# HongwenZhang/DaNet-DensePose2SMPL

Hardware: AMD Instinct MI355X
Metric: images/sec fwd+bwd HRNet-W48+SMPL+IUV 256x256 bs32/GPU (higher is better)
Workload: dtype bf16; 1 GPU; full DaNet train step (HRNet-W48 + global and part-wise IUV heads + regressor nets + SMPL LBS (2 forward + 1 backward; the 2 label-side forwards belong to the untimed batch prologue) + IUV render + losses, fwd+bwd+Adam), 256x256, 32 img/GPU; convs bf16 MFMA fp32-acc, LBS/raster/losses fp32; global_batch=32, parallelism=dp1

## Files before the change

danet-densepose2smpl_amd/_lib.py:

```python
import ctypes
import os

_HERE = os.path.dirname(os.path.abspath(__file__))
LIB_PATH = os.environ.get('DANET_LIB') or os.path.join(_HERE, 'csrc', 'libdanet_hip.so')
_lib = None

c_f = ctypes.c_void_p
c_i = ctypes.c_int
c_sz = ctypes.c_size_t
c_fl = ctypes.c_float

_SIGNATURES = {
    'danet_version': (c_i, []),
    'danet_last_error': (ctypes.c_char_p, []),
    'danet_smpl_lbs_debug': (c_i, [c_f]),
    'danet_smpl_lbs_ctx_floats': (c_sz, [c_i]),
    'danet_smpl_lbs_fwd_ws_floats': (c_sz, [c_i, c_i, c_i]),
    'danet_smpl_lbs_bwd_ws_floats': (c_sz, [c_i, c_i, c_i]),
    'danet_smpl_lbs_ticket_words': (c_sz, [c_i]),
    'danet_smpl_lbs_forward': (c_i, [c_f, c_f, c_i] + [c_f] * 9 + [c_i] * 4 + [c_f] * 5 + [c_sz, c_f, c_f]),
    'danet_smpl_lbs_backward': (c_i, [c_f, c_f, c_i] + [c_f] * 7 + [c_i] * 4 + [c_f] * 7 + [c_sz, c_f, c_i, c_f]),
    'danet_smpl_lbs_backward_fused_ok': (c_i, [c_i, c_i, c_i]),
    'danet_iuv_raster_ws_bytes': (c_sz, [c_i, c_i, c_i]),
    'danet_iuv_raster_forward': (c_i, [c_f, c_f, c_i, c_i, c_f, c_i, c_f, c_f, c_i, c_fl, c_fl, c_i, c_f, c_f, c_f, c_f, c_sz, c_f]),
# ... 44 lines not shown
    'danet_conv_wgrad3x3_pair_ok': (c_i, [c_i] * 11),
    'danet_conv_wgrad3x3_ws_floats': (c_sz, [c_i] * 7),
    'danet_conv_wgrad_multi_ws_floats': (c_sz, [c_f, c_i]),
    'danet_conv_wgrad_multi_ws_zero_from': (c_sz, [c_f, c_i]),
    'danet_conv_wgrad_multi': (c_i, [c_f, c_i, c_f, c_sz, c_fl, c_f]),
    'danet_conv_wgrad3x3_multi_ws_floats': (c_sz, [c_f, c_i]),
    'danet_conv_wgrad3x3_multi': (c_i, [c_f, c_i, c_f, c_sz, c_fl, c_f]),
    'danet_conv_wgrad3x3_kernel_id': (c_i, [c_i] * 7),
    'danet_conv_wgrad3x3': (c_i, [c_f] * 4 + [c_sz] + [c_i] * 7 + [c_fl, c_i, c_f]),
    'danet_conv_wgrad_ws_floats': (c_sz, [c_i] * 4),
    'danet_conv_wgrad_ws_floats_for': (c_sz, [c_i] * 13),
    'danet_conv_wgrad': (c_i, [c_f] * 4 + [c_sz] + [c_i] * 13 + [c_fl, c_i, c_f]),
    'danet_bn_forward': (c_i, [c_f, c_f, c_f, ctypes.c_int64, c_i] + [c_f] * 6 + [c_i, c_fl, c_fl, c_i, c_i, c_f, c_f]),
    'danet_bn_ws_floats': (c_sz, [c_i]),
    'danet_knob': (ctypes.c_long, [c_i, ctypes.c_long]),
    'danet_bn_acc_bytes': (c_i, []),
    'danet_channel_sum': (c_i, [c_f, ctypes.c_int64, c_i, c_f, c_i, c_i, c_f]),
    'danet_bn_forward_multi': (c_i, [c_f, c_i, c_fl, c_fl, c_f]),
    'danet_bn_backward_multi': (c_i, [c_f, c_i, c_f]),
    'danet_bn_backward_onepass_ok': (c_i, [c_f, c_i, c_i]),
    'danet_bn_backward_onepass_bar_words': (c_i, []),
    'danet_bn_backward_onepass': (c_i, [c_f, c_i, c_f, c_i, c_f]),
    'danet_bn_backward': (c_i, [c_f, c_f, c_f, ctypes.c_int64, c_i, c_f, c_f, c_i, c_f, c_f, c_f, c_f, c_i, c_i, c_f, c_f, c_f]),
    'danet_sum_relu_forward': (c_i, [ctypes.POINTER(ctypes.c_void_p), ctypes.POINTER(c_i), c_i, c_i, c_i, c_i, c_i, c_i, c_f, c_f]),
    'danet_sum_relu_backward': (c_i, [c_f, c_f, c_i, c_i, c_i, c_i, c_i, c_i, c_f, c_f]),
    'danet_sum_relu_backward_all': (c_i, [c_f, c_f] + [c_i] * 5 + [c_f] * 5),
    'danet_sum_relu_forward_multi': (c_i, [c_f, c_i, c_f]),
    'danet_sum_relu_backward_all_multi': (c_i, [c_f, c_i, c_f]),
    'danet_maxpool3x3s2_forward': (c_i, [c_f, c_f, c_f, c_i, c_i, c_i, c_i, c_f]),
    'danet_maxpool3x3s2_backward': (c_i, [c_f, c_f, c_f, c_i, c_i, c_i, c_i, c_f]),
    'danet_stn_gather_forward': (c_i, [c_f, c_f] + [c_i] * 8 + [c_f, c_f]),
    'danet_stn_gather_backward': (c_i, [c_f, c_f] + [c_i] * 8 + [c_f, c_f]),
    'danet_part_clean_forward': (c_i, [c_f, c_f, c_i, c_i, c_i, c_i, c_f, c_f]),
    'danet_part_clean_backward': (c_i, [c_f, c_f, c_f, c_i, c_i, c_i, c_i, c_f, c_f]),
    'danet_part_loss_forward': (c_i, [c_f] * 5 + [c_i] * 5 + [c_f, c_f]),
    'danet_part_loss_backward': (c_i, [c_f] * 6 + [c_i] * 5 + [c_f, c_f]),
    'danet_part_backward_fused': (c_i, [c_f] * 8 + [c_i] * 5 + [c_f, c_f]),
    'danet_part_gt_forward': (c_i, [c_f] * 5 + [c_i] * 4 + [c_f, c_f, c_f]),
    'danet_part_gt_backward': (c_i, [c_f] * 5 + [c_i] * 4 + [c_f, c_f]),
    'danet_iuv_global_forward': (c_i, [c_f] * 4 + [c_i, c_i] + [c_f] * 3 + [c_i] * 4 + [c_f] * 5),
    'danet_iuv_global_backward': (c_i, [c_f] * 4 + [c_i, c_i] + [c_f] * 6 + [c_i] * 4 + [c_f] * 5),
    'danet_softargmax_forward': (c_i, [c_f, c_i, c_i, c_i, c_i, c_i, c_fl, c_f, c_f, c_f]),
    'danet_softargmax_backward': (c_i, [c_f, c_i, c_i, c_i, c_i, c_i, c_fl, c_f, c_f, c_f, c_f]),
    'danet_dp_point_losses_rows': (c_i, [c_i, c_i]),
    'danet_dp_point_losses_forward': (c_i, [c_f] * 4 + [c_i, c_i] + [c_f] * 8 + [c_i] * 3 + [c_f, c_f]),
    'danet_dp_point_losses_backward': (c_i, [c_f] * 4 + [c_i, c_i] + [c_f] * 9 + [c_i] * 3 + [c_f] * 5),
# ... 259 lines not shown
```

danet-densepose2smpl_amd/csrc/build.py:

```python
import os
import subprocess
import sys
from concurrent.futures import ThreadPoolExecutor

HERE = os.path.dirname(os.path.abspath(__file__))
ROOT = os.path.dirname(os.path.dirname(HERE))
LIB = os.path.join(HERE, 'libdanet_hip.so')
ARCH = 'gfx950'

MFMA_VGPR = ['-mllvm', '-amdgpu-mfma-vgpr-form']
UNITS = {
    'capi.hip': [],
    'smpl_lbs.hip': [],
    'iuv_raster.hip': ['-ffp-contract=off'],
    'geometry.hip': [],
    'conv_igemm.hip': MFMA_VGPR,
    'conv_wgrad.hip': MFMA_VGPR,
    'conv_wgrad3x3.hip': MFMA_VGPR,
    'conv_wgrad_rows.hip': MFMA_VGPR,
    'conv3x3.hip': MFMA_VGPR,
    'conv3x3s.hip': MFMA_VGPR,
    'conv_fast.hip': MFMA_VGPR,
    'conv_g3.hip': MFMA_VGPR,
    'conv_pw.hip': MFMA_VGPR,
    'conv_pw_wgrad.hip': MFMA_VGPR,
    'conv3x3a.hip': [],
    'conv_stem_dgrad.hip': [],
    'conv_stem.hip': [],
    'conv_f32.hip': ['-ffp-contract=off'],
    'conv_f32m.hip': MFMA_VGPR,
    'part_ops.hip': [],
    'part_gt.hip': [],
    'iuv_ops.hip': [],
    'dp_losses.hip': ['-ffp-contract=off'],
    'loss_ops.hip': [],
    'adam.hip': [],
    'norm_act.hip': [],
    'norm_act_f32.hip': [],
    'stn.hip': [],
    'pool.hip': [],
    'glue.hip': [],
    'gcn_tail.hip': [],
    'lstm_tree.hip': [],
    'vis_ops.hip': ['-ffp-contract=off'],
    'eval_ops.hip': [],
    'coco_ops.hip': [],
    'input_ops.hip': ['-ffp-contract=off'],
    'train_vis.hip': ['-ffp-contract=off'],
# ... 51 lines not shown
```

danet-densepose2smpl_amd/csrc/conv_common.h:

```cpp
#pragma once
#include <hip/hip_runtime.h>

namespace danet_conv {

typedef unsigned short bf16_t;
typedef __attribute__((ext_vector_type(8))) __bf16 bf16x8;
typedef __attribute__((ext_vector_type(4))) float f32x4;

typedef __attribute__((ext_vector_type(2))) float f32x2_;
typedef __attribute__((ext_vector_type(2))) __bf16 bf16x2_;
__device__ inline unsigned f2bf_pk(float lo, float hi) {
    return __builtin_bit_cast(unsigned, __builtin_convertvector(f32x2_{lo, hi}, bf16x2_));
}
__device__ inline bf16_t f2bf(float f) { return (bf16_t)(f2bf_pk(f, 0.f) & 0xffffu); }
__device__ inline float bf2f(bf16_t h) { return __uint_as_float((unsigned)h << 16); }

constexpr int BN_NCOPY = 32;
#ifndef DANET_BN_NCOPY_DIV
#define DANET_BN_NCOPY_DIV 2
#endif
__host__ __device__ inline int bn_ncopy(int C) {
    const int n = (C <= 64 ? 32 : (C <= 128 ? 16 : (C <= 256 ? 8 : 4))) / DANET_BN_NCOPY_DIV;
    return n < 4 ? 4 : n;
}

#ifdef DANET_BN_ACC32
typedef float bn_acc_t;
#else
typedef double bn_acc_t;
#endif
constexpr int BN_ACC_FLOATS = (int)(sizeof(bn_acc_t) / sizeof(float));
__device__ inline void bn_acc_add(float* ws, int rep, int which, int Ctot, int c, float v) {
    bn_acc_t* const p = reinterpret_cast<bn_acc_t*>(ws) + ((size_t)(rep % bn_ncopy(Ctot)) * 2 + which) * Ctot + c;
    __hip_atomic_fetch_add((__attribute__((address_space(1))) bn_acc_t*)p, (bn_acc_t)v, __ATOMIC_RELAXED, __HIP_MEMORY_SCOPE_AGENT);
}

struct BnApply {
    const bf16_t* res; bf16_t* out;
    const float* gamma; const float* beta;
    float* running_mean; float* running_var;
    float* saved;
    unsigned char* mask;
    int relu;
    float momentum, eps;
    unsigned* bar;
};

struct ConvP {
    const bf16_t* x; const bf16_t* w; const float* bias; void* y;
    int B, H, W, Cin, OH, OW, Cout;
    int R, S, stride, pad, dil, groups, transposed;
    int Cin_g, Cout_g, Cout_pad, K, Kp;
    int relu, out_fp32, sshift, parity;
    float* stats;
    long M;
    const bf16_t* bn_x; const bf16_t* bn_y; const float* bn_saved; float* bn_red;
    int bn_gate;
    long x_bytes, y_bytes;
// ... 41 lines not shown
```

danet-densepose2smpl_amd/csrc/conv_pw_wgrad.hip:

```cpp
#include "common.h"
#include "conv_common.h"

namespace {

using namespace danet_conv;

typedef __attribute__((ext_vector_type(2))) unsigned v2u;
constexpr int OOB = 0x7fffffff;
constexpr int PWG_KS = 32;
constexpr int PWG_NPM = 16;
constexpr int PWG_MAXPIECES = 4;

__device__ inline v2u tr_read(unsigned lds_byte_addr) {
    v2u r;
    asm volatile("ds_read_b64_tr_b16 %0, %1" : "=v"(r) : "v"(lds_byte_addr) : "memory");
    return r;
}

struct PwgP {
    const bf16_t* x; const bf16_t* dy; float* part;
    int M, K, N;
    int KB, NB;
    int nsplit, ksplit;
    int msplit, nchunks;
// ... 279 lines not shown
            used += ((size_t)p.msplit * j.Cout * j.Cin + 15) / 16 * 16;
            const size_t l = pwg_lds(j.Cout, j.Cin, pl.nkc);
            if (l > lds) lds = l;
            ++mp.n; ++rp.n;
        }
        const dim3 grid((unsigned)mp.start[mp.n]);
#define PWG_CASE(A_, B_, C_) if (pl0.nbw_t == A_ && pl0.kbw_t == B_ && pl0.nkc == C_) { \
            if (int e = danet::raise_dynamic_lds<&conv_pw_wgrad_kernel<A_, B_, C_>>(96 * 1024, "conv_pw_wgrad_kernel")) return e; \
            hipLaunchKernelGGL((conv_pw_wgrad_kernel<A_, B_, C_>), grid, dim3(256), lds, st, mp); } else
        PWG_CASE(1, 1, 2) PWG_CASE(1, 2, 2) PWG_CASE(1, 4, 2) PWG_CASE(1, 8, 2)
        PWG_CASE(2, 1, 2) PWG_CASE(2, 2, 2) PWG_CASE(2, 4, 2)
        PWG_CASE(4, 1, 2) PWG_CASE(4, 2, 2)
        PWG_CASE(1, 1, 1) PWG_CASE(1, 2, 1) PWG_CASE(1, 4, 1) PWG_CASE(1, 8, 1) PWG_CASE(1, 16, 1)
        PWG_CASE(2, 1, 1) PWG_CASE(2, 2, 1) PWG_CASE(2, 4, 1) PWG_CASE(2, 8, 1) PWG_CASE(4, 1, 1) PWG_CASE(4, 2, 1) PWG_CASE(4, 4, 1)
        return -1;
#undef PWG_CASE
        DANET_CHECK_LAUNCH("conv_pw_wgrad_kernel");
        hipLaunchKernelGGL(conv_pw_wgrad_reduce_kernel, dim3((unsigned)danet::cdiv(rp.start[rp.n] * 8, 256)), dim3(256), 0, st, rp);
        DANET_CHECK_LAUNCH("conv_pw_wgrad_reduce_kernel");
    }
    return 0;
}

}

long danet_conv::conv_pw_wgrad_knob(long enable) {
    const long prev = g_pwg_on ? 1 : 0;
    if (enable >= 0) g_pwg_on = enable != 0;
    return prev;
}
```

danet-densepose2smpl_amd/csrc/norm_act.hip:

```cpp
#include "common.h"
#include "conv_common.h"
#include "grid_barrier.h"

namespace {

using namespace danet_conv;

constexpr int NCOPY = danet_conv::BN_NCOPY;
constexpr int VW = 4;

#ifdef NA_F32
typedef float elem_t;
constexpr int ES = 4;
constexpr int MSH = 4;
#define NA_NAME(n) n##_f32
#else
typedef bf16_t elem_t;
constexpr int ES = 2;
constexpr int MSH = 3;
#define NA_NAME(n) n
#endif

struct Vec { float v[VW]; };

// ... 355 lines not shown
    float mean[VW], invstd[VW], k0[VW], m1[VW], m2[VW], sc[VW], sh[VW];
#pragma unroll
    for (int j = 0; j < VW; ++j) {
        mean[j] = saved[c0 + j]; invstd[j] = saved[C + c0 + j];
        k0[j] = (gamma ? gamma[c0 + j] : 1.f) * invstd[j];
        sc[j] = invstd[j] * (gamma ? gamma[c0 + j] : 1.f);
        sh[j] = fmaf(-mean[j], sc[j], beta ? beta[c0 + j] : 0.f);
        const float s0 = sStat[0][c0 + j], s1 = sStat[1][c0 + j];
        m1[j] = s0 * inv_count; m2[j] = s1 * inv_count;
        if (bid == 0 && t < fm.CV && dparam) { dparam[c0 + j] = s0; dparam[C + c0 + j] = s1; }
    }
    while (it.more()) {
        Vec d[UNR], gm[UNR];
        int oo[UNR];
#pragma unroll
        for (int u = 0; u < UNR; ++u) {
            oo[u] = of[u];
#pragma unroll
            for (int j = 0; j < VW; ++j) {
                const bool on = !relu || (mask_mode == 0 ? o[u].v[j] > 0.f : mask_mode == 1 ? ((mb[u] >> j) & 1) != 0
                                                                                             : fmaf(a[u].v[j], sc[j], sh[j]) > 0.f);
                const float gv = on ? g[u].v[j] : 0.f;
                gm[u].v[j] = gv;
                d[u].v[j] = k0[j] * (gv - m1[j] - (a[u].v[j] - mean[j]) * invstd[j] * m2[j]);
            }
        }
        it.next();
        if (it.more()) fetch();
#pragma unroll
        for (int u = 0; u < UNR; ++u) {
            if (dres) stv(drr, oo[u], gm[u]);
            stv(dxr, oo[u], d[u]);
        }
    }
}
__device__ __forceinline__ void bn_bwd_apply_body(
    const int bid, const elem_t* __restrict__ dy, const elem_t* __restrict__ x, const elem_t* __restrict__ y, const FlatMap& fm,
    const float* __restrict__ saved, const float* __restrict__ gamma, const bn_acc_t* __restrict__ red,
    int Cst, float inv_count, int relu, elem_t* __restrict__ dx, elem_t* __restrict__ dres, float* __restrict__ dparam,
    int mask_mode, const unsigned char* __restrict__ mask, const float* __restrict__ beta)
{
    __shared__ float sStat[2][SLAB];
    switch (relu ? mask_mode : 3) {
        case 0: bn_bwd_apply_body_g<0>(bid, dy, x, y, fm, saved, gamma, red, Cst, inv_count, dx, dres, dparam, mask, beta, sStat); break;
        case 1: bn_bwd_apply_body_g<1>(bid, dy, x, y, fm, saved, gamma, red, Cst, inv_count, dx, dres, dparam, mask, beta, sStat); break;
        case 2: bn_bwd_apply_body_g<2>(bid, dy, x, y, fm, saved, gamma, red, Cst, inv_count, dx, dres, dparam, mask, beta, sStat); break;
        default: bn_bwd_apply_body_g<3>(bid, dy, x, y, fm, saved, gamma, red, Cst, inv_count, dx, dres, dparam, mask, beta, sStat); break;
// ... 527 lines not shown
            DANET_CHECK_LAUNCH("bn_bwd_reduce_multi_kernel");
        }
        hipLaunchKernelGGL(bn_bwd_apply_multi_kernel, dim3(m.start[ns]), dim3(256), 0, st, m);
        DANET_CHECK_LAUNCH("bn_bwd_apply_multi_kernel");
        return DANET_OK;
    }
    for (int c0 = 0; c0 < C; c0 += SLAB) {
        const int Cs = C - c0 < SLAB ? C - c0 : SLAB;
        FlatMap fm; int grid;
        DANET_CHECK_ARG(make_map(M, C, c0, Cs, &fm, &grid) == 0, "bn_backward: C=%d (M=%ld) unsupported: channels must be a multiple of 4 and the tensor < 2 GB", C, (long)M);
        if (ws_is_zero != 2) {
            hipLaunchKernelGGL(bn_bwd_reduce_kernel, dim3(grid), dim3(256), 0, st, (const elem_t*)dy, (const elem_t*)x, (const elem_t*)y,
                               fm, saved + c0, C, relu, (bn_acc_t*)red_ws + c0, mask_mode, (const unsigned char*)relu_mask,
                               gamma ? gamma + c0 : nullptr, beta ? beta + c0 : nullptr);
            DANET_CHECK_LAUNCH("bn_bwd_reduce_kernel");
        }
        hipLaunchKernelGGL(bn_bwd_apply_kernel, dim3(grid), dim3(256), 0, st, (const elem_t*)dy, (const elem_t*)x, (const elem_t*)y,
                           fm, saved + c0, gamma ? gamma + c0 : nullptr, (const bn_acc_t*)red_ws + c0, C, 1.0f / (float)M, relu, (elem_t*)dx, (elem_t*)dres,
                           dparam ? dparam + c0 : nullptr, mask_mode, (const unsigned char*)relu_mask, beta ? beta + c0 : nullptr);
        DANET_CHECK_LAUNCH("bn_bwd_apply_kernel");
    }
    return DANET_OK;
}

extern "C" int NA_NAME(danet_channel_sum)(const void* x, int64_t M, int C, double* out, int out_is_zero, int ncopy, void* stream)
{
    DANET_ENTER();
    DANET_CHECK_ARG(x && out && M > 0 && C > 0 && C % VW == 0 && ncopy >= 1 && ncopy <= 64, "channel_sum: bad arguments (C=%d must be a multiple of %d)", C, VW);
    hipStream_t st = (hipStream_t)stream;
    if (!out_is_zero) {
        hipError_t err = danet::zero_async(out, sizeof(double) * (size_t)C * ncopy, st);
        if (err != hipSuccess) return danet::fail(DANET_ERR_HIP, "channel_sum: memset: %s", hipGetErrorString(err));
    }
    for (int c0 = 0; c0 < C; c0 += SLAB) {
        const int Cs = C - c0 < SLAB ? C - c0 : SLAB;
        FlatMap fm; int grid;
        DANET_CHECK_ARG(make_map(M, C, c0, Cs, &fm, &grid) == 0, "channel_sum: C=%d (M=%ld) unsupported", C, (long)M);
        const int cap = ncopy >= 4 ? 1024 : 256;
        if (grid > cap) { grid = cap; fm.rstep = (int)((long)fm.span * grid / fm.CV); }
        hipLaunchKernelGGL(channel_sum_kernel, dim3(grid), dim3(256), 0, st, (const elem_t*)x, fm, out + c0, ncopy, C);
        DANET_CHECK_LAUNCH("channel_sum_kernel");
    }
    return DANET_OK;
}

extern "C" int NA_NAME(danet_sum_relu_forward)(const void* const* terms , const int* shifts , int nterms,
// ... 259 lines not shown
```

danet-densepose2smpl_amd/nn.py:

```python
import contextlib
import ctypes

import os
import sys
import torch
import torch.nn as nn
import torch.nn.functional as F

from . import _lib
from . import conv as _conv
from ._lib import ptr, check, stream
from .conv import Conv2d, conv2d, nhwc_bf16, nhwc_as, nhwc_act, _empty_nhwc, nptr, ARENA


def _k(L, name, dtype):
    return getattr(L, name + '_f32' if dtype == torch.float32 else name)


RELU_MASK = bool(int(os.environ.get('DANET_BN_RELU_MASK', '1')))


ONEPASS = bool(int(os.environ.get('DANET_BN_ONEPASS', '1')))
ONEPASS_STREAM = None
ONEPASS_MAX_BLOCKS = 0
# ... 329 lines not shown
        return (self.running_mean, self.running_var) if self.track_running_stats else (None, None)

    def forward(self, x, res=None, relu=False, link=None):
        training, fused = self._prologue(x)
        return BatchNormActFunction.apply(x, res, self.weight, self.bias, *self._running(), training, self._momentum(), self.eps, relu,
                                          fused, link if training else None)

    def forward_padded(self, x, d, relu=False, res=None, padded=None):
        C = self.num_features
        training, fused = self._prologue(x)
        rm = rv = None
        if self.track_running_stats:
            pad = getattr(self, '_stat_pad', None)
            if pad is None or pad[0].shape[0] != C + d or pad[0].device != x.device or self.running_mean.data_ptr() != pad[0].data_ptr():
                rm, rv = torch.zeros(C + d, device=x.device), torch.ones(C + d, device=x.device)
                rm[:C].copy_(self.running_mean); rv[:C].copy_(self.running_var)
                self._stat_pad = (rm, rv)
                self._buffers['running_mean'], self._buffers['running_var'] = rm[:C], rv[:C]
            rm, rv = self._stat_pad
        gamma, beta = padded if padded is not None else (F.pad(self.weight, (0, d)), F.pad(self.bias, (0, d)))
        return BatchNormActFunction.apply(x, res, gamma, beta, rm, rv, training, self._momentum(), self.eps, relu, fused, None)


def _shared_launch(bns, max_n):
    if not (1 <= len(bns) <= max_n and all(b.training and b.affine and b.num_features <= 1024 for b in bns)):
        return None
    mom, eps = {b._momentum() for b in bns}, {b.eps for b in bns}
    return (mom.pop(), eps.pop()) if len(mom) == 1 and len(eps) == 1 else None


class MultiBatchNormFunction(torch.autograd.Function):

    @staticmethod
    def forward(ctx, static, *tensors):
        L = _lib.lib()
        n, relu, momentum, eps, rms, rvs, fused, links = static[:8]
        done = static[8] if len(static) > 8 else None
        relus = list(relu) if isinstance(relu, (list, tuple)) else [bool(relu)] * n
        xs = [nhwc_act(t) for t in tensors[:n]]
        dt = xs[0].dtype
        ress = [None if t is None else nhwc_as(t, dt) for t in tensors[n:2 * n]]
        gammas = [t.detach().float().contiguous() for t in tensors[2 * n:3 * n]]
        betas = [t.detach().float().contiguous() for t in tensors[3 * n:4 * n]]
        if done is not None:
            ys, saveds, masks = [d[0] for d in done], [d[1] for d in done], [d[2] for d in done]
            _conv.FUSION['bn_forward_in_conv_launch'] += n
# ... 410 lines not shown
```

danet-densepose2smpl_amd/smpl_regressor.py:

```python
import numpy as np
import torch
import torch.nn as nn
import torch.nn.functional as F

from . import assets
from . import gcn_tail as _gcn_tail
from . import glue as _glue
from .config import cfg
from .gcn import GCN, adjacency, normalize_digraph, normalize_undigraph
from .geometry import perspective_projection, rot6d_to_rotmat
from .iuv_estimator import SMPL_PARENTS, SMPL_CHILDREN, DP2SMPL_MAPPING
from .lstm_tree import CHAINS as LSTM_CHAINS, LimbLSTM, lstm_tree
from .nn import Conv2d, BatchNorm2d, SideBranch, side_streams
from .resnet import SmplResNet, LimbResLayers
from .smpl import SMPL


class _StemNet(nn.Module):

    def __init__(self, in_channels, resnet):
        super().__init__()
        self.add_module('0', Conv2d(in_channels, 64, 1, bias=False))
        self.add_module('1', BatchNorm2d(64))
        self.add_module('3', resnet)

    def __getitem__(self, i):
        return self._modules[str(i)]

    def forward(self, x):
        return self._modules['3'](self._modules['1'](self._modules['0'](x), relu=True))


class _MlpBnRelu(nn.Module):

    def __init__(self, cin, mid, cout):
        super().__init__()
        self.add_module('0', Conv2d(cin, mid, 1))
        self.add_module('1', BatchNorm2d(mid))
        self.add_module('3', Conv2d(mid, cout, 1))
        self.add_module('4', BatchNorm2d(cout))

    def __getitem__(self, i):
        return self._modules[str(i)]

    def forward(self, x):
        m = self._modules
        return m['4'](m['3'](m['1'](m['0'](x), relu=True)), relu=True)


def _tree_levels():
    depth = [0] * 24
    for j in range(1, 24):
        depth[j] = depth[SMPL_PARENTS[j]] + 1
# ... 377 lines not shown
```

include/danet_hip.h:

```cpp
#ifndef DANET_HIP_H
#define DANET_HIP_H

#include <stddef.h>
#include <stdint.h>

#ifdef __cplusplus
extern "C" {
#endif

#define DANET_OK 0
#define DANET_ERR_ARG (-1)
#define DANET_ERR_HIP (-2)
#define DANET_ERR_WORKSPACE (-3)

int danet_version(void);
const char* danet_last_error(void);

size_t danet_smpl_lbs_ctx_floats(int B);
size_t danet_smpl_lbs_fwd_ws_floats(int B, int V, int NE);
size_t danet_smpl_lbs_bwd_ws_floats(int B, int V, int NB);
size_t danet_smpl_lbs_ticket_words(int B);

int danet_smpl_lbs_forward(const float* betas, const float* rotmats, int B,
                           const float* v_template, const float* shapedirs, const float* posedirs,
// ... 209 lines not shown
int danet_conv_wgrad3x3(const void* x, const void* dy, float* dw, float* ws, size_t ws_floats,
                        int B, int H, int W, int Cin, int Cout, int groups, int stride, float beta, int phase , void* stream);
int danet_conv_wgrad_rows_ok(int B, int H, int W, int Cin, int OH, int OW, int Cout, int R, int S, int stride, int pad, int dil, int groups);
size_t danet_conv_wgrad_rows_ws_floats(int B, int OH, int OW, int Cin, int Cout, int R, int S, int groups);
int danet_conv_wgrad_rows(const void* x, const void* dy, float* dw, float* ws, size_t ws_floats,
                          int B, int H, int W, int Cin, int OH, int OW, int Cout,
                          int R, int S, int stride, int pad, int groups, float beta, void* stream);
size_t danet_conv_wgrad_ws_floats(int Cout, int Cin_g, int R, int S);
size_t danet_conv_wgrad_ws_floats_for(int B, int H, int W, int Cin, int OH, int OW, int Cout, int R, int S, int stride, int pad, int dil, int groups);
int danet_conv_wgrad(const void* x, const void* dy, float* dw, float* ws, size_t ws_floats,
                     int B, int H, int W, int Cin, int OH, int OW, int Cout,
                     int R, int S, int stride, int pad, int dil, int groups, float beta, int ws_is_zero, void* stream);

int danet_bn_forward(const void* x, const void* res, void* y, int64_t M, int C,
                     const float* gamma, const float* beta, float* running_mean, float* running_var,
                     float* saved, float* sums_ws, int ws_is_zero, float momentum, float eps, int training, int relu,
                     void* relu_mask, void* stream);
size_t danet_bn_ws_floats(int C);
int danet_bn_acc_bytes(void);
int danet_bn_backward(const void* dy, const void* x, const void* y, int64_t M, int C,
                      const float* gamma, const float* saved, int relu,
                      void* dx, void* dres, float* dparam, float* red_ws, int ws_is_zero,
                      int mask_mode, const void* relu_mask, const float* beta, void* stream);
int danet_bn_forward_multi(const void* jobs, int n, float momentum, float eps, void* stream);
int danet_bn_backward_multi(const void* jobs, int n, void* stream);
int danet_bn_backward_onepass_bar_words(void);
int danet_bn_backward_onepass_ok(const void* jobs, int n, int max_blocks);
int danet_bn_backward_onepass(const void* jobs, int n, void* bar, int max_blocks, void* stream);
int danet_channel_sum(const void* x, int64_t M, int C, double* out, int out_is_zero, int ncopy, void* stream);
int danet_channel_sum_f32(const void* x, int64_t M, int C, double* out, int out_is_zero, int ncopy, void* stream);
int danet_sum_relu_forward(const void* const* terms, const int* shifts, int nterms,
                           int B, int H, int W, int C, int relu, void* y, void* stream);
int danet_sum_relu_backward(const void* gy, const void* y, int B, int H, int W, int C, int shift, int relu,
                            void* d_term, void* stream);
int danet_sum_relu_forward_multi(const void* jobs, int n, void* stream);
int danet_sum_relu_backward_all_multi(const void* jobs, int n, void* stream);
int danet_sum_relu_backward_all(const void* gy, const void* y, int B, int H, int W, int C, int relu,
                                void* d0, void* d1, void* d2, void* d3, void* stream);
int danet_bn_forward_f32(const void* x, const void* res, void* y, int64_t M, int C,
                         const float* gamma, const float* beta, float* running_mean, float* running_var,
                         float* saved, float* sums_ws, int ws_is_zero, float momentum, float eps, int training, int relu,
                         void* relu_mask, void* stream);
int danet_bn_backward_f32(const void* dy, const void* x, const void* y, int64_t M, int C,
                          const float* gamma, const float* saved, int relu,
                          void* dx, void* dres, float* dparam, float* red_ws, int ws_is_zero,
                          int mask_mode, const void* relu_mask, const float* beta, void* stream);
// ... 108 lines not shown
```

Before: 1327 images/sec.

## Fuse BN backward with 1x1 conv dgrad and wgrad in regressor head

Adds a new HIP kernel that computes the BatchNorm(+ReLU) input gradient on the fly and feeds it straight into MFMA-based dgrad and split-M wgrad for a 1x1 conv with 64 output channels. A new autograd function and the pw_conv_bn helper route the regressor head's conv-BN-ReLU pair through it. This removes the round trip of writing the BN gradient to memory and reading it back in separate dgrad and wgrad kernels, and cuts launches. In exchange it adds a partial-sum workspace and a reduction kernel, and it only applies to a narrow set of shapes, with Cin up to 96.

```diff
diff --git a/danet-densepose2smpl_amd/_lib.py b/danet-densepose2smpl_amd/_lib.py
--- a/danet-densepose2smpl_amd/_lib.py
+++ b/danet-densepose2smpl_amd/_lib.py
@@ -90,6 +90,10 @@
     'danet_bn_backward_onepass_bar_words': (c_i, []),
     'danet_bn_backward_onepass': (c_i, [c_f, c_i, c_f, c_i, c_f]),
     'danet_bn_backward': (c_i, [c_f, c_f, c_f, ctypes.c_int64, c_i, c_f, c_f, c_i, c_f, c_f, c_f, c_f, c_i, c_i, c_f, c_f, c_f]),
+    'danet_pw_bn_backward_ok': (c_i, [ctypes.c_int64, c_i, c_i, c_i, c_i, c_i]),
+    'danet_pw_bn_backward_ws_floats': (c_sz, [ctypes.c_int64, c_i]),
+    'danet_pw_bn_backward': (c_i, [c_f, c_f, c_f, c_f, c_i, c_f, c_f, c_f, c_f, c_i, ctypes.c_int64, c_i, c_i, c_i, c_f, c_f, c_fl, c_f,
+                                   c_f, c_sz, c_f]),
     'danet_sum_relu_forward': (c_i, [ctypes.POINTER(ctypes.c_void_p), ctypes.POINTER(c_i), c_i, c_i, c_i, c_i, c_i, c_i, c_f, c_f]),
     'danet_sum_relu_backward': (c_i, [c_f, c_f, c_i, c_i, c_i, c_i, c_i, c_i, c_f, c_f]),
     'danet_sum_relu_backward_all': (c_i, [c_f, c_f] + [c_i] * 5 + [c_f] * 5),
diff --git a/danet-densepose2smpl_amd/csrc/build.py b/danet-densepose2smpl_amd/csrc/build.py
--- a/danet-densepose2smpl_amd/csrc/build.py
+++ b/danet-densepose2smpl_amd/csrc/build.py
@@ -24,6 +24,7 @@
     'conv_g3.hip': MFMA_VGPR,
     'conv_pw.hip': MFMA_VGPR,
     'conv_pw_wgrad.hip': MFMA_VGPR,
+    'conv_pw_bnbwd.hip': MFMA_VGPR,
     'conv3x3a.hip': [],
     'conv_stem_dgrad.hip': [],
     'conv_stem.hip': [],
diff --git a/danet-densepose2smpl_amd/csrc/conv_common.h b/danet-densepose2smpl_amd/csrc/conv_common.h
--- a/danet-densepose2smpl_amd/csrc/conv_common.h
+++ b/danet-densepose2smpl_amd/csrc/conv_common.h
@@ -34,6 +34,14 @@
     bn_acc_t* const p = reinterpret_cast<bn_acc_t*>(ws) + ((size_t)(rep % bn_ncopy(Ctot)) * 2 + which) * Ctot + c;
     __hip_atomic_fetch_add((__attribute__((address_space(1))) bn_acc_t*)p, (bn_acc_t)v, __ATOMIC_RELAXED, __HIP_MEMORY_SCOPE_AGENT);
 }
+
+__device__ __forceinline__ float bn_bwd_dx(float gv, float a, float k0, float m1, float m2, float mean, float invstd) {
+    return k0 * (gv - m1 - (a - mean) * invstd * m2);
+}
+
+int bn_bwd_reduce_launch(const void* dy, const void* x, long M, int C, const float* gamma, const float* beta, const float* saved,
+                         int relu, int mask_mode, float* red_ws, void* stream);
+int conv_pw_wgrad_reduce_launch(const float* part, float* dw, int msplit, long total, float beta, void* stream);
 
 struct BnApply {
     const bf16_t* res; bf16_t* out;
diff --git a/danet-densepose2smpl_amd/csrc/conv_pw_bnbwd.hip b/danet-densepose2smpl_amd/csrc/conv_pw_bnbwd.hip
--- /dev/null
+++ b/danet-densepose2smpl_amd/csrc/conv_pw_bnbwd.hip
@@ -0,0 +1,264 @@
+#include "common.h"
+#include "conv_common.h"
+
+namespace {
+
+using namespace danet_conv;
+
+typedef __attribute__((ext_vector_type(2))) unsigned v2u;
+constexpr int OOB = 0x7fffffff;
+constexpr int PB_CH = 64;
+constexpr int PB_N = 64;
+constexpr int PB_PXY = PB_N * 2 + 32;
+constexpr int PB_MAXSPLIT = 1024;
+
+__device__ inline v2u tr_read(unsigned lds_byte_addr) {
+    v2u r;
+    asm volatile("ds_read_b64_tr_b16 %0, %1" : "=v"(r) : "v"(lds_byte_addr) : "memory");
+    return r;
+}
+
+struct PbP {
+    const bf16_t* da; const bf16_t* c; const bf16_t* x; const float* w;
+    const float* gamma; const float* beta; const float* saved; const bn_acc_t* red;
+    bf16_t* dx; float* part; float* dparam;
+    int M, K, Kw;
+    int msplit, nchunks;
+    int y_bytes, x_bytes;
+    float inv_count;
+};
+
+template <int KB, bool RELU>
+__global__ __launch_bounds__(256) void conv_pw_bnbwd_kernel(PbP p)
+{
+    extern __shared__ __attribute__((aligned(16))) unsigned char smem[];
+    const int bx = blockIdx.x;
+    const int t = threadIdx.x, lane = t & 63;
+    const int wave = __builtin_amdgcn_readfirstlane(t >> 6);
+    const int li = lane & 15, lg = lane >> 4;
+    const int K = p.K;
+    constexpr int PXX = KB * 32 + 32;
+    constexpr int YB = PB_CH * PB_PXY, BUF = YB + PB_CH * PXX;
+    constexpr int XP = (PB_CH * KB * 2 + 255) / 256;
+
+    const int per = (p.nchunks + p.msplit - 1) / p.msplit;
+    const int c_begin = bx * per, c_end = min(p.nchunks, c_begin + per);
+
+    const int c8 = t & 7;
+    const __amdgpu_buffer_rsrc_t gr = __builtin_amdgcn_make_buffer_rsrc(const_cast<bf16_t*>(p.da), 0, p.y_bytes, 0x00020000);
+    const __amdgpu_buffer_rsrc_t cr = __builtin_amdgcn_make_buffer_rsrc(const_cast<bf16_t*>(p.c), 0, p.y_bytes, 0x00020000);
+    const __amdgpu_buffer_rsrc_t xr = __builtin_amdgcn_make_buffer_rsrc(const_cast<bf16_t*>(p.x), 0, p.x_bytes, 0x00020000);
+    constexpr int K8 = KB * 2;
+    int xrel[XP], xlds[XP], xq[XP];
+#pragma unroll
+    for (int u = 0; u < XP; ++u) {
+        const int pc = t + u * 256;
+        const int q = pc / K8, k8 = pc - q * K8;
+        const bool in = pc < PB_CH * K8;
+        xrel[u] = (in && k8 * 8 < K) ? (q * K + k8 * 8) * 2 : OOB;
+        xlds[u] = in ? q * PXX + k8 * 16 : -1;
+        xq[u] = q;
+    }
+    uint4 gst[2], cst[2], xst[XP];
+    auto fetch = [&](int ch) {
+        const int m0 = ch * PB_CH;
+#pragma unroll
+        for (int u = 0; u < 2; ++u) {
+            const int q = (t >> 3) + 32 * u;
+            const int off = m0 + q < p.M ? ((m0 + q) * PB_N + c8 * 8) * 2 : OOB;
+            gst[u] = __builtin_bit_cast(uint4, __builtin_amdgcn_raw_buffer_load_b128(gr, off, 0, 0));
+            cst[u] = __builtin_bit_cast(uint4, __builtin_amdgcn_raw_buffer_load_b128(cr, off, 0, 0));
+        }
+#pragma unroll
+        for (int u = 0; u < XP; ++u)
+            xst[u] = __builtin_bit_cast(uint4, __builtin_amdgcn_raw_buffer_load_b128(xr, (xrel[u] != OOB && m0 + xq[u] < p.M) ? m0 * K * 2 + xrel[u] : OOB, 0, 0));
+    };
+    if (c_begin < c_end) fetch(c_begin);
+
+    {
+        float* const sStat = reinterpret_cast<float*>(smem);
+        if (t < 2 * PB_N) {
+            const int ncopy = bn_ncopy(PB_N);
+            bn_acc_t s = 0;
+            for (int r = 0; r < ncopy; ++r) s += p.red[(size_t)r * 2 * PB_N + t];
+            sStat[t] = (float)s;
+        }
+        __syncthreads();
+    }
+    float mean[8], invstd[8], k0[8], m1[8], m2[8], sc[8], sh[8];
+    {
+        const float* const sStat = reinterpret_cast<const float*>(smem);
+#pragma unroll
+        for (int j = 0; j < 8; ++j) {
+            const int ch = c8 * 8 + j;
+            const float gm = p.gamma ? p.gamma[ch] : 1.f;
+            mean[j] = p.saved[ch]; invstd[j] = p.saved[PB_N + ch];
+            k0[j] = gm * invstd[j];
+            sc[j] = invstd[j] * gm;
+            sh[j] = fmaf(-mean[j], sc[j], p.beta ? p.beta[ch] : 0.f);
+            const float s0 = sStat[ch], s1 = sStat[PB_N + ch];
+            m1[j] = s0 * p.inv_count; m2[j] = s1 * p.inv_count;
+            if (bx == 0 && t < 8 && p.dparam) { p.dparam[ch] = s0; p.dparam[PB_N + ch] = s1; }
+        }
+        __syncthreads();
+    }
+
+    bf16x8 wf[KB][2];
+#pragma unroll
+    for (int nb = 0; nb < KB; ++nb)
+#pragma unroll
+        for (int ks = 0; ks < 2; ++ks) {
+            const int cin = nb * 16 + li;
+            uint4 raw;
+            unsigned h[8];
+#pragma unroll
+            for (int j = 0; j < 8; ++j) h[j] = cin < p.Kw ? (unsigned)f2bf(p.w[(size_t)(ks * 32 + lg * 8 + j) * p.Kw + cin]) : 0u;
+            raw.x = h[0] | (h[1] << 16); raw.y = h[2] | (h[3] << 16); raw.z = h[4] | (h[5] << 16); raw.w = h[6] | (h[7] << 16);
+            wf[nb][ks] = __builtin_bit_cast(bf16x8, raw);
+        }
+
+    f32x4 acc[KB];
+#pragma unroll
+    for (int j = 0; j < KB; ++j) acc[j] = f32x4{0.f, 0.f, 0.f, 0.f};
+    const unsigned aoff = (unsigned)((lg * 8 + (li >> 2)) * PB_PXY + (wave * 16 + 4 * (li & 3)) * 2);
+    unsigned boff[KB];
+#pragma unroll
+    for (int j = 0; j < KB; ++j) boff[j] = (unsigned)((lg * 8 + (li >> 2)) * PXX + (j * 16 + 4 * (li & 3)) * 2);
+    const unsigned doff = (unsigned)((wave * 16 + li) * PB_PXY + lg * 16);
+
+    auto commit = [&](int buf, int ch) {
+        unsigned char* const base = smem + buf * BUF;
+        const int m0 = ch * PB_CH;
+#pragma unroll
+        for (int u = 0; u < 2; ++u) {
+            const int q = (t >> 3) + 32 * u;
+            const unsigned gw[4] = {gst[u].x, gst[u].y, gst[u].z, gst[u].w}, cw[4] = {cst[u].x, cst[u].y, cst[u].z, cst[u].w};
+            float d[8];
+#pragma unroll
+            for (int j = 0; j < 8; ++j) {
+                const float g = __uint_as_float((j & 1) ? (gw[j >> 1] & 0xffff0000u) : (gw[j >> 1] << 16));
+                const float a = __uint_as_float((j & 1) ? (cw[j >> 1] & 0xffff0000u) : (cw[j >> 1] << 16));
+                const bool on = !RELU || fmaf(a, sc[j], sh[j]) > 0.f;
+                d[j] = bn_bwd_dx(on ? g : 0.f, a, k0[j], m1[j], m2[j], mean[j], invstd[j]);
+            }
+            uint4 o;
+            o.x = f2bf_pk(d[0], d[1]); o.y = f2bf_pk(d[2], d[3]); o.z = f2bf_pk(d[4], d[5]); o.w = f2bf_pk(d[6], d[7]);
+            if (m0 + q >= p.M) o = uint4{0u, 0u, 0u, 0u};
+            *reinterpret_cast<uint4*>(base + q * PB_PXY + c8 * 16) = o;
+        }
+#pragma unroll
+        for (int u = 0; u < XP; ++u)
+            if (xlds[u] >= 0) *reinterpret_cast<uint4*>(base + YB + xlds[u]) = xst[u];
+    };
+
+    int buf = 0;
+    for (int ch = c_begin; ch < c_end; ++ch) {
+        commit(buf, ch);
+        __syncthreads();
+        if (ch + 1 < c_end) fetch(ch + 1);
+        const unsigned ybase = (unsigned)(buf * BUF), xbase = ybase + (unsigned)YB;
+#pragma unroll
+        for (int ks = 0; ks < 2; ++ks) {
+            const unsigned yk = ybase + (unsigned)(ks * 32 * PB_PXY), xk = xbase + (unsigned)(ks * 32 * PXX);
+            v2u alo, ahi, blo[KB], bhi[KB];
+            alo = tr_read(yk + aoff); ahi = tr_read(yk + aoff + 4 * PB_PXY);
+#pragma unroll
+            for (int j = 0; j < KB; ++j) { blo[j] = tr_read(xk + boff[j]); bhi[j] = tr_read(xk + boff[j] + 4 * PXX); }
+            asm volatile("s_waitcnt lgkmcnt(0)" ::: "memory");
+            __builtin_amdgcn_sched_barrier(0);
+            const uint4 araw = {alo.x, alo.y, ahi.x, ahi.y};
+            const bf16x8 a = __builtin_bit_cast(bf16x8, araw);
+#pragma unroll
+            for (int j = 0; j < KB; ++j) {
+                const uint4 braw = {blo[j].x, blo[j].y, bhi[j].x, bhi[j].y};
+                acc[j] = __builtin_amdgcn_mfma_f32_16x16x32_bf16(a, __builtin_bit_cast(bf16x8, braw), acc[j], 0, 0, 0);
+            }
+        }
+        {
+            const uint4 d0 = *reinterpret_cast<const uint4*>(smem + ybase + doff), d1 = *reinterpret_cast<const uint4*>(smem + ybase + doff + 64);
+            const bf16x8 b0 = __builtin_bit_cast(bf16x8, d0), b1 = __builtin_bit_cast(bf16x8, d1);
+            const int px = ch * PB_CH + wave * 16 + li;
+            bf16_t* const row = p.dx + (size_t)px * K;
+#pragma unroll
+            for (int nb = 0; nb < KB; ++nb) {
+                f32x4 o = __builtin_amdgcn_mfma_f32_16x16x32_bf16(wf[nb][0], b0, f32x4{0.f, 0.f, 0.f, 0.f}, 0, 0, 0);
+                o = __builtin_amdgcn_mfma_f32_16x16x32_bf16(wf[nb][1], b1, o, 0, 0, 0);
+                const int cin = nb * 16 + 4 * lg;
+                if (px < p.M && cin < K) *reinterpret_cast<uint2*>(row + cin) = uint2{f2bf_pk(o[0], o[1]), f2bf_pk(o[2], o[3])};
+            }
+        }
+        buf ^= 1;
+    }
+    float* const dst = p.part + (size_t)bx * PB_N * K;
+#pragma unroll
+    for (int j = 0; j < KB; ++j) {
+        const int cin = j * 16 + li;
+        if (cin >= K) continue;
+#pragma unroll
+        for (int r = 0; r < 4; ++r) dst[(size_t)(wave * 16 + lg * 4 + r) * K + cin] = acc[j][r];
+    }
+}
+
+int pb_msplit(long M, int K) {
+    const long nchunks = (M + PB_CH - 1) / PB_CH;
+    long ms = (long)danet::compute_units() * ((K + 15) / 16 <= 2 ? 3 : 2);
+    if (ms > nchunks / 8) ms = nchunks / 8;
+    if (ms > PB_MAXSPLIT) ms = PB_MAXSPLIT;
+    if (ms < 1) ms = 1;
+    return (int)ms;
+}
+
+}
+
+extern "C" int danet_pw_bn_backward_ok(int64_t M, int Cin, int Cout, int relu, int mask_mode, int has_res)
+{
+    if (Cout != PB_N || Cin <= 0 || Cin % 8 != 0 || Cin > 96 || has_res) return 0;
+    if (relu && mask_mode != 2) return 0;
+    if (M <= 0 || M * (Cin > PB_N ? Cin : PB_N) * 2 >= (1LL << 31) - (64 << 20)) return 0;
+    return 1;
+}
+
+extern "C" size_t danet_pw_bn_backward_ws_floats(int64_t M, int Cin)
+{
+    if (M <= 0 || Cin <= 0) return 0;
+    return (size_t)PB_MAXSPLIT * PB_N * Cin;
+}
+
+extern "C" int danet_pw_bn_backward(const void* da, const void* c, const void* x0, const float* w, int Cin_w,
+                                    const float* gamma, const float* beta, const float* saved, float* red, int red_zero,
+                                    int64_t M, int Cin, int Cout, int relu, void* dx0, float* dW, float dW_beta, float* dparam,
+                                    float* workspace, size_t ws_floats, void* stream)
+{
+    DANET_ENTER();
+    DANET_CHECK_ARG(da && c && x0 && w && saved && red && dx0 && dW && workspace, "pw_bn_backward: bad arguments");
+    DANET_CHECK_ARG(danet_pw_bn_backward_ok(M, Cin, Cout, relu, 2, 0), "pw_bn_backward: M=%ld Cin=%d Cout=%d is not the fused kernel's case", (long)M, Cin, Cout);
+    DANET_CHECK_ARG(Cin_w > 0 && Cin_w <= Cin, "pw_bn_backward: the weight has %d input channels, the tensors %d", Cin_w, Cin);
+    DANET_CHECK_ARG(ws_floats >= danet_pw_bn_backward_ws_floats(M, Cin), "pw_bn_backward: workspace too small");
+    hipStream_t st = (hipStream_t)stream;
+    if (red_zero != 2) {
+        if (!red_zero) {
+            hipError_t e = danet::zero_async(red, danet_bn_ws_floats(PB_N) * sizeof(float), st);
+            if (e != hipSuccess) return danet::fail(DANET_ERR_HIP, "pw_bn_backward: memset: %s", hipGetErrorString(e));
+        }
+        if (int e = danet_conv::bn_bwd_reduce_launch(da, c, M, PB_N, gamma, beta, saved, relu, 2, red, stream)) return e;
+    }
+    PbP p;
+    p.da = (const bf16_t*)da; p.c = (const bf16_t*)c; p.x = (const bf16_t*)x0; p.w = w;
+    p.gamma = gamma; p.beta = beta; p.saved = saved; p.red = (const bn_acc_t*)red;
+    p.dx = (bf16_t*)dx0; p.part = workspace; p.dparam = dparam;
+    p.M = (int)M; p.K = Cin; p.Kw = Cin_w;
+    p.nchunks = (int)((M + PB_CH - 1) / PB_CH); p.msplit = pb_msplit(M, Cin);
+    p.y_bytes = (int)(M * PB_N * 2); p.x_bytes = (int)(M * Cin * 2);
+    p.inv_count = 1.0f / (float)M;
+    const int KB = (Cin + 15) / 16;
+    const size_t lds = (size_t)2 * PB_CH * (PB_PXY + KB * 32 + 32);
+    const dim3 grid((unsigned)p.msplit);
+#define PB_CASE(KB_) if (KB == KB_) { \
+        if (relu) hipLaunchKernelGGL((conv_pw_bnbwd_kernel<KB_, true>), grid, dim3(256), lds, st, p); \
+        else hipLaunchKernelGGL((conv_pw_bnbwd_kernel<KB_, false>), grid, dim3(256), lds, st, p); } else
+    PB_CASE(1) PB_CASE(2) PB_CASE(3) PB_CASE(4) PB_CASE(5) PB_CASE(6)
+    return danet::fail(DANET_ERR_ARG, "pw_bn_backward: no instantiation for Cin=%d", Cin);
+#undef PB_CASE
+    DANET_CHECK_LAUNCH("conv_pw_bnbwd_kernel");
+    return danet_conv::conv_pw_wgrad_reduce_launch(workspace, dW, p.msplit, (long)PB_N * Cin, dW_beta, stream);
+}
diff --git a/danet-densepose2smpl_amd/csrc/conv_pw_wgrad.hip b/danet-densepose2smpl_amd/csrc/conv_pw_wgrad.hip
--- a/danet-densepose2smpl_amd/csrc/conv_pw_wgrad.hip
+++ b/danet-densepose2smpl_amd/csrc/conv_pw_wgrad.hip
@@ -325,6 +325,14 @@
     return 0;
 }
 
+int conv_pw_wgrad_reduce_launch(const float* part, float* dw, int msplit, long total, float beta, void* stream) {
+    PwgRed rp;
+    rp.n = 1; rp.beta = beta; rp.part[0] = part; rp.dw[0] = dw; rp.msplit[0] = msplit; rp.start[0] = 0; rp.start[1] = total;
+    hipLaunchKernelGGL(conv_pw_wgrad_reduce_kernel, dim3((unsigned)danet::cdiv(total * 8, 256)), dim3(256), 0, (hipStream_t)stream, rp);
+    DANET_CHECK_LAUNCH("conv_pw_wgrad_reduce_kernel");
+    return 0;
+}
+
 }
 
 long danet_conv::conv_pw_wgrad_knob(long enable) {
diff --git a/danet-densepose2smpl_amd/csrc/norm_act.hip b/danet-densepose2smpl_amd/csrc/norm_act.hip
--- a/danet-densepose2smpl_amd/csrc/norm_act.hip
+++ b/danet-densepose2smpl_amd/csrc/norm_act.hip
@@ -401,7 +401,7 @@
                                                                                              : fmaf(a[u].v[j], sc[j], sh[j]) > 0.f);
                 const float gv = on ? g[u].v[j] : 0.f;
                 gm[u].v[j] = gv;
-                d[u].v[j] = k0[j] * (gv - m1[j] - (a[u].v[j] - mean[j]) * invstd[j] * m2[j]);
+                d[u].v[j] = danet_conv::bn_bwd_dx(gv, a[u].v[j], k0[j], m1[j], m2[j], mean[j], invstd[j]);
             }
         }
         it.next();
@@ -975,6 +975,21 @@
     }
     return DANET_OK;
 }
+
+#ifndef NA_F32
+int danet_conv::bn_bwd_reduce_launch(const void* dy, const void* x, long M, int C, const float* gamma, const float* beta, const float* saved,
+                                     int relu, int mask_mode, float* red_ws, void* stream)
+{
+    DANET_CHECK_ARG(dy && x && saved && red_ws && M > 0 && C > 0 && C <= SLAB && (!relu || mask_mode == 2),
+                    "bn_bwd_reduce_launch: one slab, ReLU gate recomputed from x");
+    FlatMap fm; int grid;
+    DANET_CHECK_ARG(make_map(M, C, 0, C, &fm, &grid) == 0, "bn_bwd_reduce_launch: C=%d (M=%ld) unsupported", C, M);
+    hipLaunchKernelGGL(bn_bwd_reduce_kernel, dim3(grid), dim3(256), 0, (hipStream_t)stream, (const elem_t*)dy, (const elem_t*)x, (const elem_t*)nullptr,
+                       fm, saved, C, relu, (bn_acc_t*)red_ws, mask_mode, (const unsigned char*)nullptr, gamma, beta);
+    DANET_CHECK_LAUNCH("bn_bwd_reduce_kernel");
+    return DANET_OK;
+}
+#endif
 
 extern "C" int NA_NAME(danet_channel_sum)(const void* x, int64_t M, int C, double* out, int out_is_zero, int ncopy, void* stream)
 {
diff --git a/danet-densepose2smpl_amd/nn.py b/danet-densepose2smpl_amd/nn.py
--- a/danet-densepose2smpl_amd/nn.py
+++ b/danet-densepose2smpl_amd/nn.py
@@ -375,6 +375,92 @@
         return BatchNormActFunction.apply(x, res, gamma, beta, rm, rv, training, self._momentum(), self.eps, relu, fused, None)
 
 
+PW_BN_BWD = bool(int(os.environ.get('DANET_PW_BN_BWD', '1')))
+
+
+class PwConvBnFunction(torch.autograd.Function):
+
+    @staticmethod
+    def forward(ctx, x, weight, gamma, beta, running_mean, running_var, momentum, eps, relu, wpad):
+        L = _lib.lib()
+        x = nhwc_bf16(x)
+        B, Cin, H, W = x.shape
+        Cout = weight.shape[0]
+        M = B * H * W
+        sums = ARENA.zeros(L.danet_bn_ws_floats(Cout), x.device)
+        c = _conv._conv_fwd_raw(x, _conv.pack_weight(weight, 1, 0, 0, wpad), None, B, H, W, Cin, H, W, Cout, 1, 1, 1, 0, 1, 1, False, False, False, sums)
+        y, saved, mask = _bn_fwd_outputs(c, None, True, relu)
+        g, b = gamma.detach().float().contiguous(), beta.detach().float().contiguous()
+        check(L.danet_bn_forward(nptr(c), None, nptr(y), M, Cout, ptr(g), ptr(b), ptr(running_mean), ptr(running_var), ptr(saved), ptr(sums), 2,
+                                 float(momentum), float(eps), 1, int(relu), ptr(mask), stream()), 'danet_bn_forward')
+        ctx.save_for_backward(x, c, weight, g, b, saved)
+        ctx.relu, ctx.wpad = bool(relu), wpad
+        if _conv.TRACE is not None:
+            _conv.TRACE.append(('bn', tuple(c.shape), y.float().abs().mean()))
+        y._bn_ctx = _conv.BnCtx(c, bool(relu), saved, mask, _bn_relu_gate(True, relu, False)[1])
+        return y
+
+    @staticmethod
+    def backward(ctx, gy):
+        L = _lib.lib()
+        x, c, weight, g, b, saved = ctx.saved_tensors
+        red = getattr(gy, '_bn_red', None)
+        gy = nhwc_bf16(gy)
+        B, Cin, H, W = x.shape
+        Cout = c.shape[1]
+        M = B * H * W
+        _conv.FUSION['bn_bwd_reduce_fused' if red is not None else 'bn_bwd_reduce_own'] += 1
+        _conv.FUSION['pw_bn_bwd_fused'] += 1
+        if red is not None:
+            red_zero = 2
+        else:
+            red, red_zero = _bn_scratch(L.danet_bn_ws_floats(Cout), x.device)
+        dparam = torch.empty(2, Cout, dtype=torch.float32, device=x.device)
+        dx = _empty_nhwc(B, Cin, H, W, torch.bfloat16, x.device)
+        gw = _conv.new_wgrad(weight, tuple(weight.shape), x.device)
+        gwp = gw if ctx.wpad is None else torch.empty(Cout, Cin, 1, 1, dtype=torch.float32, device=x.device)
+        w = weight.detach()
+        if w.dtype != torch.float32 or not w.is_contiguous():
+            w = w.float().contiguous()
+        nws = L.danet_pw_bn_backward_ws_floats(M, Cin)
+        ws = torch.empty(nws, dtype=torch.float32, device=x.device)
+        with _conv._timed('conv_pw_bnbwd_kernel', 4.0 * M * Cout * Cin, ('dgrad+wgrad', B, H, W, Cin, Cout, 1, 1, 1)):
+            check(L.danet_pw_bn_backward(nptr(gy), nptr(c), nptr(x), ptr(w), weight.shape[1], ptr(g), ptr(b), ptr(saved), ptr(red), int(red_zero),
+                                         M, Cin, Cout, int(ctx.relu), nptr(dx), ptr(gwp), 0.0, ptr(dparam), ptr(ws), nws, stream()),
+                  'danet_pw_bn_backward')
+        if ctx.wpad is not None:
+            from .glue import crop_into
+            crop_into([gwp], [(1, Cout, Cin, 1)], [(1, weight.shape[0], weight.shape[1], 1)], [gw])
+        if _conv.TRACE is not None:
+            _conv.TRACE.append(('pw_bn_bwd' + ('+red' if red_zero == 2 else ''), tuple(x.shape), dx.float().abs().mean()))
+        return dx, gw, dparam[1], dparam[0], None, None, None, None, None, None
+
+
+def pw_conv_bn(conv, bn, x, relu=False):
+    if not (isinstance(conv, Conv2d) and isinstance(bn, BatchNorm2d)):
+        return bn(conv(x), relu=relu)
+    w = conv.weight
+    ok = PW_BN_BWD and conv.training and bn.training and torch.is_grad_enabled() and not _conv.fp32_mode() and x.is_cuda and x.dim() == 4 and \
+        conv.bias is None and not conv.out_fp32 and conv.groups == 1 and tuple(conv.kernel_size) == (1, 1) and tuple(conv.stride) == (1, 1) and \
+        tuple(conv.padding) == (0, 0) and bn.weight is not None and bn.bias is not None and _conv.FUSE_BN_STATS and \
+        w.is_cuda and w.dtype == torch.float32 and w.is_contiguous()
+    if ok:
+        mode = _bn_relu_gate(True, relu, False)[1]
+        padc, pad_x, padn = _conv.channel_padding(x.shape[1], w.shape[1], w.shape[0], 1)
+        B, _, H, W = x.shape
+        cin = x.shape[1] + (padc if pad_x else 0)
+        ok = padn == 0 and cin == w.shape[1] + padc and \
+            bool(_lib.lib().danet_pw_bn_backward_ok(B * H * W, cin, w.shape[0], int(relu), mode, 0))
+    if not ok:
+        return bn(conv(x), relu=relu)
+    if pad_x:
+        x = _conv._pad_channels_nhwc(x)
+    bn._count()
+    _conv.FUSION['bn_stats_fused'] += 1
+    return PwConvBnFunction.apply(x, w, bn.weight, bn.bias, *bn._running(), bn._momentum(), bn.eps, bool(relu),
+                                  (w.shape[0], w.shape[1] + padc) if padc else None)
+
+
 def _shared_launch(bns, max_n):
     if not (1 <= len(bns) <= max_n and all(b.training and b.affine and b.num_features <= 1024 for b in bns)):
         return None
diff --git a/danet-densepose2smpl_amd/smpl_regressor.py b/danet-densepose2smpl_amd/smpl_regressor.py
--- a/danet-densepose2smpl_amd/smpl_regressor.py
+++ b/danet-densepose2smpl_amd/smpl_regressor.py
@@ -11,7 +11,7 @@
 from .geometry import perspective_projection, rot6d_to_rotmat
 from .iuv_estimator import SMPL_PARENTS, SMPL_CHILDREN, DP2SMPL_MAPPING
 from .lstm_tree import CHAINS as LSTM_CHAINS, LimbLSTM, lstm_tree
-from .nn import Conv2d, BatchNorm2d, SideBranch, side_streams
+from .nn import Conv2d, BatchNorm2d, SideBranch, side_streams, pw_conv_bn
 from .resnet import SmplResNet, LimbResLayers
 from .smpl import SMPL
 
@@ -28,7 +28,7 @@
         return self._modules[str(i)]
 
     def forward(self, x):
-        return self._modules['3'](self._modules['1'](self._modules['0'](x), relu=True))
+        return self._modules['3'](pw_conv_bn(self._modules['0'], self._modules['1'], x, relu=True))
 
 
 class _MlpBnRelu(nn.Module):
diff --git a/include/danet_hip.h b/include/danet_hip.h
--- a/include/danet_hip.h
+++ b/include/danet_hip.h
@@ -255,6 +255,12 @@
                       const float* gamma, const float* saved, int relu,
                       void* dx, void* dres, float* dparam, float* red_ws, int ws_is_zero,
                       int mask_mode, const void* relu_mask, const float* beta, void* stream);
+int danet_pw_bn_backward_ok(int64_t M, int Cin, int Cout, int relu, int mask_mode, int has_res);
+size_t danet_pw_bn_backward_ws_floats(int64_t M, int Cin);
+int danet_pw_bn_backward(const void* da, const void* c, const void* x0, const float* w, int Cin_w,
+                         const float* gamma, const float* beta, const float* saved, float* red, int red_zero,
+                         int64_t M, int Cin, int Cout, int relu, void* dx0, float* dW, float dW_beta, float* dparam,
+                         float* workspace, size_t ws_floats, void* stream);
 int danet_bn_forward_multi(const void* jobs, int n, float momentum, float eps, void* stream);
 int danet_bn_backward_multi(const void* jobs, int n, void* stream);
 int danet_bn_backward_onepass_bar_words(void);
```

Result: no change. 1338 images/sec (median of 6 runs) (+0.8%).
